# matter-labs/era-zkevm_test_harness

Hardware: AMD Instinct MI355X
Metric: base-layer circuits/sec (2^20 rows); full-block synth wall-time 1/8 GPU (higher is better)
Workload: dtype u64 (Goldilocks, p = 2^64 - 2^32 + 1)

## Files before the change

era_zkevm_test_harness_amd/csrc/ram_circuit_kernels.cuh:

```cuda
#pragma once
#include "../../include/zkw_ram_circuit_spec.h"
#include "../../include/zkw_decommit_sorter_circuit_spec.h"
#include "../../include/zkw_events_sorter_circuit_spec.h"
#include "ram_kernels.cuh"
#include "public_input_kernels.cuh"
#include "closed_form_kernels.cuh"

namespace zkw {

struct SynthJob {
    const zkw_ram_instance* inst;
    const zkw_mem_query* sorted_q;
    const zkw_mem_query* unsorted_q;
    const u64* unsorted_caps;
    const u64* sorted_caps;
    const u64* u_mark;
    const u64* s_mark;
    const u64* challenges;
    const u64* lhs_z;
    const u64* rhs_z;
    u64 n_block;
    u64* trace;
    u32* hist;
    u32* nd_tiles;
    const u64* public_input;
    const zkw_ram_instance* first_inst;
    u32 tail_clean;
};

constexpr int ROW_SLOTS[RC_NUM_ROW_TYPES] = RC_ROW_NUM_SLOTS_INIT;
constexpr int ROW_LOOKUPS[RC_NUM_ROW_TYPES] = RC_ROW_NUM_LOOKUPS_INIT;
static_assert(ROW_SLOTS[RC_ROW_PU] == 133 && ROW_SLOTS[RC_ROW_PS] == 130, "Poseidon2 rows: 130 gate variables (+3 spare in PU)");
static_assert(ROW_LOOKUPS[RC_ROW_PU] == 12 && ROW_LOOKUPS[RC_ROW_PS] == 12 && ROW_LOOKUPS[RC_ROW_A] == 12 &&
              ROW_LOOKUPS[RC_ROW_B] == 12 && ROW_LOOKUPS[RC_ROW_C] == 8 && ROW_LOOKUPS[RC_ROW_D] == 0,
              "lookup cells per cycle (56) are hard-wired in the fill kernels");
constexpr int LOOKUPS_PER_CYCLE = 56;

__device__ __forceinline__ u64 inv_or_zero(u64 x) { return gl::canon(x) ? gl::inv(x) : 0; }

struct RegsIn {
    const u64* uh;
    const u64* sh;
    u32 len;
};
// ... 79 lines not shown
    memset(&c.q, 0, sizeof c.q);
    memset(&c.pq, 0, sizeof c.pq);
#pragma unroll
    for (int k = 0; k < 8; k++) c.es[k] = 0;
    if (c.can_pop) {
        load_query(job.sorted_q + first + i, c.q);
        encode_mem_query(c.q, c.es);
    }
    if (i == 0) {
        const zkw_ram_fsm& f = in->hidden_fsm_input;
        c.pq.timestamp = f.previous_sorting_key[0]; c.pq.index = f.previous_sorting_key[1]; c.pq.page = f.previous_sorting_key[2];
        for (int k = 0; k < 8; k++) c.pq.value[k] = f.previous_value[k];
        c.pq.value_is_pointer = f.previous_is_ptr ? 1 : 0;
    } else if (i - 1 < m) {
        load_query(job.sorted_q + first + i - 1, c.pq);
    }
    u64 pe[8];
    encode_mem_query(c.pq, pe);
#pragma unroll
    for (int k = 0; k < 5; k++) c.p_val[k] = pe[3 + k];
    c.p_ptr = c.pq.value_is_pointer ? 1 : 0;
}

__device__ __forceinline__ u64 acc_before(const u64* z, size_t first, size_t m, u32 i, u64 fsm_in) {
    return i == 0 ? fsm_in : z[first + (i - 1 < m ? i - 1 : m - 1)];
}

__device__ __forceinline__ void fill_row_A(const SynthJob& job, u32 i, u32 capacity, size_t n_rows, const zkw_mem_query& q,
                                           const u64 eu[8], const u64 es[8], u32* sh_hist) {
    u64* trace = job.trace;
    const size_t row = (size_t)RC_ROW_A * RC_REGION_STRIDE(capacity) + i;
    if (i < capacity) {
        const zkw_ram_instance* in = job.inst;
        const size_t first = in->first_item, m = in->num_items, n_total = job.n_block;
        const bool can_pop = i < m;
        const u64 rw = q.rw_flag ? 1 : 0, ptr = q.value_is_pointer ? 1 : 0;
#pragma unroll
        for (int k = 0; k < 8; k++) { TR(RC_A_eu0 + k, row) = eu[k]; TR(RC_A_ts + k, row) = es[k]; }
        for (int r = 0; r < 2; r++) {
            const u64* ch = job.challenges + 9 * r;
            u64 lc = ch[8], rc = ch[8];
#pragma unroll
            for (int k = 0; k < 8; k++) {
                lc = gl::add(lc, gl::mul(eu[k], ch[k]));
                rc = gl::add(rc, gl::mul(es[k], ch[k]));
                __builtin_amdgcn_sched_barrier(0);
            }
            const u64 pl = acc_before(job.lhs_z + (size_t)r * n_total, first, m, i, in->hidden_fsm_input.lhs_accumulator[r]);
            const u64 pr = acc_before(job.rhs_z + (size_t)r * n_total, first, m, i, in->hidden_fsm_input.rhs_accumulator[r]);
            const u64 nl = gl::canon(gl::mul(pl, lc)), nr = gl::canon(gl::mul(pr, rc));
            const int o = r * (RC_A_lc1 - RC_A_lc0);
#pragma unroll
            for (int k = 1; k < 9; k++) TR(RC_A_G_c0_1 + (k - 1) + r * (RC_A_G_c1_1 - RC_A_G_c0_1), row) = ch[k];
            __builtin_amdgcn_sched_barrier(0);
            TR(RC_A_lc0 + o, row) = gl::canon(lc); TR(RC_A_P_lhs0 + o, row) = pl; TR(RC_A_nl0 + o, row) = nl;
            TR(RC_A_lhs0 + o, row) = can_pop ? nl : pl;
            TR(RC_A_rc0 + o, row) = gl::canon(rc); TR(RC_A_P_rhs0 + o, row) = pr; TR(RC_A_nr0 + o, row) = nr;
            TR(RC_A_rhs0 + o, row) = can_pop ? nr : pr;
            __builtin_amdgcn_sched_barrier(0);
        }
        TR(RC_A_rw, row) = rw; TR(RC_A_ptr, row) = ptr; TR(RC_A_idx, row) = q.index;
        TR(RC_A_v2, row) = q.value[2]; TR(RC_A_v3, row) = q.value[3]; TR(RC_A_v0, row) = q.value[0];
        TR(RC_A_v5_b3c, row) = q.value[5] >> 24; TR(RC_A_can_pop, row) = can_pop ? 1 : 0;
        put_bytes(trace, n_rows, row, RC_A_v2_b0, q.value[2]);
        put_bytes(trace, n_rows, row, RC_A_v3_b0, q.value[3]);
        put_bytes(trace, n_rows, row, RC_A_v5_b0, q.value[5]);
        hist_bytes(sh_hist, q.value[2]); hist_bytes(sh_hist, q.value[3]); hist_bytes(sh_hist, q.value[5]);
        constexpr int NA = ROW_SLOTS[RC_ROW_A];
        if (!job.tail_clean) {
            for (int col = NA; col < RC_G; col++) TR(col, row) = 0;
            for (int col = RC_G + 12; col < RC_G + RC_L; col++) TR(col, row) = 0;
        }
    } else if (i < RC_REGION_STRIDE(capacity)) {
        if (!job.tail_clean) zero_gap_row(trace, n_rows, row);
    }
}

__device__ __forceinline__ void fill_row_B(const SynthJob& job, u32 i, u32 capacity, size_t n_rows, const zkw_mem_query& q,
                                           const u64 es[8], u32* sh_hist) {
    u64* trace = job.trace;
    const size_t row = (size_t)RC_ROW_B * RC_REGION_STRIDE(capacity) + i;
    if (i < capacity) {
        const zkw_ram_instance* in = job.inst;
// ... 286 lines not shown
        const size_t per = (n_pairs + TAIL_CHUNKS - 1) / TAIL_CHUNKS, lo = ch * per, hi = lo + per < n_pairs ? lo + per : n_pairs;
        ulonglong2* c2 = reinterpret_cast<ulonglong2*>(trace + (size_t)col * n_rows + bnd);
        const ulonglong2 z = make_ulonglong2(0, 0);
        for (size_t k = lo + threadIdx.x; k < hi; k += 256) c2[k] = z;
        return;
    }
    u64* m = trace + (size_t)RC_MULT_COL * n_rows;
    const size_t per = (n_rows + TAIL_CHUNKS - 1) / TAIL_CHUNKS, lo = ch * per, hi = lo + per < n_rows ? lo + per : n_rows;
    for (size_t r = lo + threadIdx.x; r < (job.tail_clean && hi > 256 ? (lo < 256 ? 256 : lo) : hi); r += 256) {
        u64 v = 0;
        if (r < 256) {
            v = job.hist[r];
            if (r == 0) v += (u64)RC_L * n_rows - (u64)LOOKUPS_PER_CYCLE * capacity - RC_CF_LOOKUP_CELLS;
        }
        m[r] = v;
    }
}

static __constant__ rc_link c_links[RC_NUM_LINKS] = RC_LINKS_INIT;
static __constant__ uint8_t c_is_poseidon[RC_NUM_ROW_TYPES] = RC_ROW_IS_POSEIDON_INIT;
ZKW_CF_TABLES(RC, rc)

__device__ __forceinline__ void ram_fill_register_rows(const SynthJob& job, u32 capacity, size_t n_rows) {
    const u64* lhs_z_all = job.lhs_z;
    const u64* rhs_z_all = job.rhs_z;
    const size_t n_total = job.n_block;
    u64* trace = job.trace;
    const zkw_ram_instance* in = job.inst;
    const zkw_ram_fsm& fi = in->hidden_fsm_input;
    const size_t first = in->first_item, m = in->num_items;
    const size_t bin = (size_t)RC_BOUNDARY_ROW(capacity) + RC_ROWOFF_BND_IN, bout = bin - RC_ROWOFF_BND_IN + RC_ROWOFF_BND_OUT;
    const RegsIn ri = regs_in(in);
    for (int k = 0; k < 12; k++) { TR(RC_BND_IN_uh0 + k, bin) = ri.uh[k]; TR(RC_BND_IN_sh0 + k, bin) = ri.sh[k]; }
    TR(RC_BND_IN_len_u, bin) = ri.len; TR(RC_BND_IN_len_s, bin) = ri.len;
    for (int r = 0; r < 2; r++) { TR(RC_BND_IN_lhs0 + r, bin) = fi.lhs_accumulator[r]; TR(RC_BND_IN_rhs0 + r, bin) = fi.rhs_accumulator[r]; }
    zkw_mem_query pq;
    memset(&pq, 0, sizeof pq);
    for (int k = 0; k < 8; k++) pq.value[k] = fi.previous_value[k];
    u64 pe[8];
    encode_mem_query(pq, pe);
    TR(RC_BND_IN_ts, bin) = fi.previous_sorting_key[0]; TR(RC_BND_IN_idx, bin) = fi.previous_sorting_key[1];
    TR(RC_BND_IN_page, bin) = fi.previous_sorting_key[2];
    TR(RC_BND_IN_es3, bin) = pe[3]; TR(RC_BND_IN_es4, bin) = pe[4]; TR(RC_BND_IN_es5, bin) = pe[5];
    TR(RC_BND_IN_es6, bin) = pe[6]; TR(RC_BND_IN_v4, bin) = pe[7];
    TR(RC_BND_IN_ptr, bin) = fi.previous_is_ptr ? 1 : 0; TR(RC_BND_IN_cnt, bin) = fi.num_nondeterministic_writes;
    for (int r = 0; r < 2; r++)
        for (int k = 1; k < 9; k++) TR(RC_BND_IN_G_c0_1 + 8 * r + (k - 1), bin) = job.challenges[9 * r + k];
    const size_t last = first + m - 1;
    const bool padded = m < capacity;
    const u64 len_out = (u64)ri.len - m;
    for (int k = 0; k < 12; k++) {
        TR(RC_BND_OUT_uh0 + k, bout) = job.u_mark[k];
        TR(RC_BND_OUT_sh0 + k, bout) = job.s_mark[k];
        TR(RC_BND_OUT_tail_u0 + k, bout) = in->unsorted_queue_initial_state.tail[k];
        TR(RC_BND_OUT_tail_s0 + k, bout) = in->sorted_queue_initial_state.tail[k];
    }
    TR(RC_BND_OUT_len_u, bout) = len_out; TR(RC_BND_OUT_len_s, bout) = len_out;
    for (int r = 0; r < 2; r++) {
        TR(RC_BND_OUT_lhs0 + r, bout) = lhs_z_all[(size_t)r * n_total + last];
        TR(RC_BND_OUT_rhs0 + r, bout) = rhs_z_all[(size_t)r * n_total + last];
    }
    zkw_mem_query lq;
    memset(&lq, 0, sizeof lq);
    if (!padded) lq = job.sorted_q[last];
    u64 le[8];
    encode_mem_query(lq, le);
    TR(RC_BND_OUT_ts, bout) = lq.timestamp; TR(RC_BND_OUT_idx, bout) = lq.index; TR(RC_BND_OUT_page, bout) = lq.page;
    TR(RC_BND_OUT_es3, bout) = le[3]; TR(RC_BND_OUT_es4, bout) = le[4]; TR(RC_BND_OUT_es5, bout) = le[5];
    TR(RC_BND_OUT_es6, bout) = le[6]; TR(RC_BND_OUT_v4, bout) = le[7];
    TR(RC_BND_OUT_ptr, bout) = lq.value_is_pointer ? 1 : 0;
    TR(RC_BND_OUT_cnt, bout) = TR(RC_C_cnt, (size_t)RC_ROW_C * RC_REGION_STRIDE(capacity) + capacity - 1);
    TR(RC_BND_OUT_completion, bout) = in->completion_flag ? 1 : 0;
    TR(RC_BND_OUT_w_end, bout) = inv_or_zero(len_out); TR(RC_BND_OUT_z_end, bout) = len_out == 0;
}

__device__ __forceinline__ void ram_value_row(u64* trace, size_t n_rows, size_t row, int v0, int b0, int e3) {
    zkw_mem_query q;
    memset(&q, 0, sizeof q);
    for (int k = 0; k < 8; k++) q.value[k] = (u32)TR(v0 + k, row);
    for (int l = 5; l < 8; l++)
        for (int k = 0; k < 4; k++) {
            const u64 b = (q.value[l] >> (8 * k)) & 0xFF;
            TR(b0 + 4 * (l - 5) + k, row) = b;
// ... 225 lines not shown
```

era_zkevm_test_harness_amd/csrc/ram_kernels.cuh:

```cuda
#pragma once
#include "../../include/zkw_types.h"
#include "poseidon2.cuh"

namespace zkw {
using gl::u32;
using gl::u64;

__device__ __forceinline__ void encode_mem_query(const zkw_mem_query& q, u64 out[8]) {
    const u32* v = q.value;
    out[0] = q.timestamp;
    out[1] = q.page;
    out[2] = (u64)q.index | ((u64)(q.rw_flag ? 1 : 0) << 32) | ((u64)(q.value_is_pointer ? 1 : 0) << 33);
    u64 b5 = v[5], b6 = v[6], b7 = v[7];
    out[3] = (u64)v[0] | ((b5 & 0xFFFFFF) << 32);
    out[4] = (u64)v[1] | ((b5 >> 24) << 32) | ((b6 & 0xFFFF) << 40);
    out[5] = (u64)v[2] | ((b6 >> 16) << 32) | ((b7 & 0xFF) << 48);
    out[6] = (u64)v[3] | ((b7 >> 8) << 32);
    out[7] = v[4];
}

static __device__ __forceinline__ void k_encode_mem(const VB& vb, const zkw_mem_query* __restrict__ q, size_t n,
                                                    u64* __restrict__ enc) {
    size_t i = (size_t)vb.x * blockDim.x + threadIdx.x;
    size_t stride = (size_t)vb.nx * blockDim.x;
// ... 415 lines not shown
    uint4 w0 = src[0], w1 = src[1], w2 = src[2];
    uint4* dq = reinterpret_cast<uint4*>(sorted_q + i);
    dq[0] = w0; dq[1] = w1; dq[2] = w2;
    zkw_mem_query m;
    uint4* dm = reinterpret_cast<uint4*>(&m);
    dm[0] = w0; dm[1] = w1; dm[2] = w2;
    if (!sorted_enc) return;
    u64 e[8];
    encode_mem_query(m, e);
    ulonglong2* o = reinterpret_cast<ulonglong2*>(sorted_enc + 8 * i);
    o[0] = make_ulonglong2(e[0], e[1]); o[1] = make_ulonglong2(e[2], e[3]);
    o[2] = make_ulonglong2(e[4], e[5]); o[3] = make_ulonglong2(e[6], e[7]);
}

struct RamBlock {
    const zkw_mem_query* sorted_q;
    const u32* sorted_perm;
    const u64* u_marks;
    const u64* s_marks;
    const u64* lhs_z;
    const u64* rhs_z;
    zkw_ram_instance* instances;
    u32* nondet_prefix;
    u64 n;
    u32 capacity;
    u32 num_nondet_heap_queries;
};

__device__ __forceinline__ void copy12(u64* dst, const u64* src) {
    for (int k = 0; k < 12; k++) dst[k] = src[k];
}

static __device__ __forceinline__ void k_ram_count_nondet(const VB& vb, const RamBlock* __restrict__ blocks) {
    const RamBlock b = blocks[vb.y];
    const u64 n_inst = (b.n + b.capacity - 1) / b.capacity;
    __shared__ u32 sh[4];
    for (u64 inst = vb.x; inst < n_inst; inst += vb.nx) {
        const u64 lo = inst * b.capacity, hi = lo + b.capacity < b.n ? lo + b.capacity : b.n;
        u32 cnt = 0;
        for (u64 i = lo + threadIdx.x; i < hi; i += blockDim.x) {
            const zkw_mem_query* q = b.sorted_q + b.sorted_perm[i];
            cnt += (q->rw_flag && q->timestamp == 0 && q->page == ZKW_BOOTLOADER_HEAP_PAGE) ? 1u : 0u;
        }
        for (int d = 32; d > 0; d >>= 1) cnt += __shfl_down(cnt, d, 64);
        if ((threadIdx.x & 63) == 0) sh[threadIdx.x >> 6] = cnt;
        __syncthreads();
// ... 36 lines not shown
        f.current_sorted_queue_state.length = (u32)(n - end);
        const zkw_mem_query* q = b.sorted_q + b.sorted_perm[l];
        f.previous_sorting_key[0] = q->timestamp; f.previous_sorting_key[1] = q->index; f.previous_sorting_key[2] = q->page;
        f.previous_full_key[0] = q->index; f.previous_full_key[1] = q->page;
        for (int k = 0; k < 8; k++) f.previous_value[k] = q->value[k];
        f.previous_is_ptr = q->value_is_pointer ? 1 : 0;
        f.num_nondeterministic_writes = nondet;
    };
    if (idx == 0) {
        for (int r = 0; r < 2; r++) { w.hidden_fsm_input.lhs_accumulator[r] = 1; w.hidden_fsm_input.rhs_accumulator[r] = 1; }
    } else {
        fill(w.hidden_fsm_input, lo, nondet_before);
    }
    fill(w.hidden_fsm_output, hi, nondet_before + b.nondet_prefix[idx]);
    if ((hi - lo) % b.capacity != 0) {
        zkw_ram_fsm& f = w.hidden_fsm_output;
        for (int k = 0; k < 3; k++) f.previous_sorting_key[k] = 0;
        for (int k = 0; k < 2; k++) f.previous_full_key[k] = 0;
        for (int k = 0; k < 8; k++) f.previous_value[k] = 0;
        f.previous_is_ptr = 0;
    }
}


static __device__ __forceinline__ void k_tails_expand(const VB& vb, const u64* __restrict__ enc, const u64* __restrict__ caps,
                                                     const u64* __restrict__ offsets, int n_queues, size_t n,
                                                     u64* __restrict__ tails) {
    const size_t i = (size_t)vb.x * blockDim.x + threadIdx.x;
    if (i >= n) return;
    int lo = 0, hi = n_queues;
    while (hi - lo > 1) {
        const int mid = (lo + hi) >> 1;
        if (offsets[mid] <= i) lo = mid; else hi = mid;
    }
    u64 s[12];
#pragma unroll
    for (int k = 0; k < 8; k++) s[k] = enc[8 * i + k];
    const bool first = offsets[lo] == i;
#pragma unroll
    for (int k = 0; k < 4; k++) s[8 + k] = first ? 0 : caps[4 * (i - 1) + k];
    p2::permute(s);
#pragma unroll
    for (int k = 0; k < 12; k++) tails[12 * i + k] = gl::canon(s[k]);
}

}
// ... 1 lines not shown
```

era_zkevm_test_harness_amd/csrc/zkw_api.hip:

```cpp
#include "zkw_ctx.h"
#include "circuit_check_host.h"
#include "closed_forms_host.h"
#include "callstack_kernels.cuh"
#include "vm_kernels.cuh"
#include "radix_sort.cuh"

static thread_local std::string g_last_error;

#undef fail
int zkw_fail(int code, const char* fmt, ...) {
    char buf[512];
    va_list ap;
    va_start(ap, fmt);
    vsnprintf(buf, sizeof buf, fmt, ap);
    va_end(ap);
    g_last_error = buf;
    return code;
}

#define fail zkw_fail

struct AllocCache {
    static constexpr size_t SMALL_MAX = size_t(256) << 20;
    static constexpr int MAX_DEV = 16;
// ... 912 lines not shown
    uint64_t offsets[2] = {0, n};
    return zkw_queue_push_chain_log_batch(ctx, enc, offsets, 1, tail_in, old_tails, new_tails);
}

struct zkw_ram_witness {
    zkw_ctx* ctx = nullptr;
    std::vector<uint64_t> offsets;
    std::vector<uint64_t> inst_offsets;
    uint32_t capacity = 0;
    size_t total = 0, n_instances = 0;
    zkw_mem_query* sorted_q = nullptr;
    bool sorted_valid = false;
    u32* perm = nullptr;
    const zkw_mem_query* unsorted_q = nullptr;
    zkw_mem_query* owned_q = nullptr;
    u64 *unsorted_enc = nullptr, *sorted_enc = nullptr;
    bool enc_valid = false;
    u64 *unsorted_caps = nullptr, *sorted_caps = nullptr, *unsorted_marks = nullptr, *sorted_marks = nullptr;
    u64 *unsorted_tails = nullptr, *sorted_tails = nullptr;
    bool tails_valid = false;
    u64 *challenges = nullptr, *lhs_z = nullptr, *rhs_z = nullptr;
    bool z_valid = false;
    u64 *zbuf_l = nullptr, *zbuf_r = nullptr;
    zkw_mem_query* sq_win = nullptr;
    size_t zcap = 0, sqcap = 0;
    zkw_ram_instance* instances = nullptr;
    u32* nondet_counts = nullptr;
    u64 *compact_forms = nullptr, *public_inputs = nullptr;

    void release() {
        void* ptrs[] = {sorted_q, perm, owned_q, unsorted_enc, sorted_enc, unsorted_caps, sorted_caps, unsorted_marks, sorted_marks,
                        unsorted_tails, sorted_tails, challenges,
                        lhs_z,    rhs_z,        instances,  nondet_counts, compact_forms, public_inputs, zbuf_l, zbuf_r, sq_win};
        for (void* p : ptrs)
            if (p) dev_free(p);
        sorted_q = nullptr;
        sorted_valid = false;
        perm = nullptr;
        owned_q = nullptr;
        unsorted_q = nullptr;
        enc_valid = false;
        unsorted_enc = sorted_enc = unsorted_tails = sorted_tails = challenges = lhs_z = rhs_z = nullptr;
        unsorted_caps = sorted_caps = unsorted_marks = sorted_marks = nullptr;
        tails_valid = false;
        z_valid = false;
        zbuf_l = zbuf_r = nullptr;
        sq_win = nullptr;
        zcap = sqcap = 0;
        instances = nullptr;
        nondet_counts = nullptr;
        compact_forms = public_inputs = nullptr;
    }
};

extern "C" void zkw_ram_witness_free(zkw_ram_witness* w);
static int ram_alloc(zkw_ram_witness* w, size_t n_blocks) {
    const size_t t = w->total, ni = w->n_instances;
    HIP_TRY(dev_malloc((void**)&w->perm, (t + 1) * sizeof(u32)));
    HIP_TRY(dev_malloc((void**)&w->unsorted_caps, (t + 1) * 4 * sizeof(u64)));
    HIP_TRY(dev_malloc((void**)&w->sorted_caps, (t + 1) * 4 * sizeof(u64)));
    HIP_TRY(dev_malloc((void**)&w->unsorted_marks, (ni + 1) * 12 * sizeof(u64)));
    HIP_TRY(dev_malloc((void**)&w->sorted_marks, (ni + 1) * 12 * sizeof(u64)));
    HIP_TRY(dev_malloc((void**)&w->challenges, (n_blocks + 1) * 18 * sizeof(u64)));
    {
        size_t max_block = 0;
        for (size_t b = 0; b + 1 < w->offsets.size(); b++) max_block = std::max(max_block, (size_t)(w->offsets[b + 1] - w->offsets[b]));
        size_t window = (size_t)1 << 26, sq_window = (size_t)1 << 22;
        if (const char* e = getenv("ZKW_Z_WINDOW_ITEMS")) window = sq_window = (size_t)strtoull(e, nullptr, 10);
        w->zcap = std::max(max_block, std::min(t, window));
        w->sqcap = std::max(max_block, std::min(t, sq_window));
        HIP_TRY(dev_malloc((void**)&w->zbuf_l, (w->zcap + 1) * 2 * sizeof(u64)));
        HIP_TRY(dev_malloc((void**)&w->zbuf_r, (w->zcap + 1) * 2 * sizeof(u64)));
        HIP_TRY(dev_malloc((void**)&w->sq_win, (w->sqcap + 1) * sizeof(zkw_mem_query)));
    }
    HIP_TRY(dev_malloc((void**)&w->instances, (ni + 1) * sizeof(zkw_ram_instance)));
    HIP_TRY(dev_malloc((void**)&w->nondet_counts, (ni + 1) * sizeof(u32)));
    HIP_TRY(dev_malloc((void**)&w->compact_forms, (ni + 1) * COMPACT_FORM_LEN * sizeof(u64)));
    HIP_TRY(dev_malloc((void**)&w->public_inputs, (ni + 1) * 4 * sizeof(u64)));
    return ZKW_OK;
}

__device__ __forceinline__ u32 block_of_position(const u64* __restrict__ offsets, int n_blocks, size_t i) {
    int lo = 0, hi = n_blocks;
    while (hi - lo > 1) {
        int mid = (lo + hi) >> 1;
        if (offsets[mid] <= i) lo = mid; else hi = mid;
    }
    return (u32)lo;
}

static __device__ __forceinline__ void k_ram_key_ranges(const VB& vb, const zkw_mem_query* __restrict__ q, size_t n, u32* __restrict__ maxima) {
    u32 t = 0, p = 0, x = 0;
    for (size_t i = (size_t)vb.x * blockDim.x + threadIdx.x; i < n; i += (size_t)vb.nx * blockDim.x) {
        t = max(t, q[i].timestamp);
        p = max(p, q[i].page);
        x = max(x, q[i].index);
    }
// ... 151 lines not shown
                      w->challenges + 18 * b};
    }
    ZKW_TRY(dev_fs(ctx, fs, 12, 9));
    w->z_valid = false;
    for (size_t b0 = 0; b0 < n_blocks;) {
        size_t b1 = b0 + 1;
        while (b1 < n_blocks && w->offsets[b1 + 1] - w->offsets[b0] <= w->zcap) b1++;
        ZKW_TRY(ram_gp_blocks(ctx, w, b0, b1, w->zbuf_l, w->zbuf_r));
        const size_t base = w->offsets[b0];
        std::vector<RamBlock> blocks(b1 - b0);
        size_t max_inst = 0;
        for (size_t b = b0; b < b1; b++) {
            const size_t lo = w->offsets[b], n = w->offsets[b + 1] - lo;
            const size_t n_inst = w->inst_offsets[b + 1] - w->inst_offsets[b];
            if (n_inst > max_inst) max_inst = n_inst;
            blocks[b - b0] = RamBlock{w->unsorted_q,
                                      w->perm + lo,
                                      w->unsorted_marks + 12 * w->inst_offsets[b],
                                      w->sorted_marks + 12 * w->inst_offsets[b],
                                      w->zbuf_l + 2 * (lo - base),
                                      w->zbuf_r + 2 * (lo - base),
                                      w->instances + w->inst_offsets[b],
                                      w->nondet_counts + w->inst_offsets[b],
                                      n,
                                      w->capacity,
                                      n_nondet ? n_nondet[b] : 0u};
        }
        RamBlock* d_blocks = nullptr;
        ZKW_TRY(ctx->upload("ram_blocks", blocks, &d_blocks));
        const unsigned gx = (unsigned)(max_inst < 64 ? max_inst : 64), gy = (unsigned)(b1 - b0);
        { Prof _p(ctx, "k_ram_count_nondet"); ZKW_LAUNCH_2D(ctx, k_ram_count_nondet, gx, gy, 256, d_blocks); }
        ZKW_TRY(launch_check("k_ram_count_nondet"));
        { Prof _p(ctx, "k_ram_instances"); ZKW_LAUNCH_2D(ctx, k_ram_instances, blocks_for(max_inst, 64), gy, 64, d_blocks); }
        ZKW_TRY(launch_check("k_ram_instances"));
        b0 = b1;
    }
    const size_t ni = w->n_instances;
    { Prof _p(ctx, "k_ram_commitments"); ZKW_LAUNCH(ctx, k_ram_commitments, blocks_for(4 * ni, 64), 64, w->instances, ni, w->compact_forms); }
    ZKW_TRY(launch_check("k_ram_commitments"));
    { Prof _p(ctx, "k_commit_encodings"); ZKW_LAUNCH(ctx, k_commit_encodings, blocks_for(ni, 64), 64, w->compact_forms, ni, (u32)COMPACT_FORM_LEN, w->public_inputs); }
    return launch_check("k_commit_encodings");
}

extern "C" int zkw_ram_build_instances_batch(zkw_ctx* ctx, const zkw_mem_query* q, const uint64_t* block_offsets,
                                             size_t n_blocks, uint32_t capacity, const uint32_t* n_nondet,
                                             zkw_ram_witness** out) {
    if (!ctx || !q || !block_offsets || !out || n_blocks == 0 || capacity == 0)
        return fail(ZKW_ERR_INVALID, "zkw_ram_build_instances_batch: bad argument");
    HIP_TRY(hipSetDevice(ctx->device));
    const uint64_t base = block_offsets[0];
    std::vector<uint64_t> offs(n_blocks + 1), ioffs(n_blocks + 1, 0);
    for (size_t b = 0; b <= n_blocks; b++) offs[b] = block_offsets[b] - base;
    for (size_t b = 0; b < n_blocks; b++) {
        if (block_offsets[b + 1] <= block_offsets[b])
            return fail(ZKW_ERR_INVALID, "block %zu is empty: the VM must have made memory requests "
                                         "(W/ram_permutation.rs:43-46)", b);
        ioffs[b + 1] = ioffs[b] + (offs[b + 1] - offs[b] + capacity - 1) / capacity;
// ... 111 lines not shown
    { Prof _p(ctx, "k_tails_expand"); ZKW_LAUNCH(ctx, k_tails_expand, blocks_for(t, 64), 64, w->sorted_enc, w->sorted_caps, d_off, nq, t, w->sorted_tails); }
    ZKW_TRY(launch_check("k_tails_expand"));
    w->tails_valid = true;
    return ZKW_OK;
}

static const void* ram_array(const zkw_ram_witness* w, int what, size_t* bytes, bool materialize = true, int* rc = nullptr) {
    const size_t t = w->total, nb = w->offsets.size() - 1;
    int st = ZKW_OK;
    const void* p = nullptr;
#define RAM_LAZY(fn, field) do { if (materialize) { st = fn(w); if (st == ZKW_OK) p = w->field; } } while (0)
    switch (what) {
        case ZKW_RAM_SORTED_QUERIES: *bytes = t * sizeof(zkw_mem_query); RAM_LAZY(ram_sorted_queries, sorted_q); break;
        case ZKW_RAM_UNSORTED_ENC: *bytes = t * 64; RAM_LAZY(ram_encodings, unsorted_enc); break;
        case ZKW_RAM_SORTED_ENC: *bytes = t * 64; RAM_LAZY(ram_encodings, sorted_enc); break;
        case ZKW_RAM_UNSORTED_TAILS: *bytes = t * 96; RAM_LAZY(ram_full_tails, unsorted_tails); break;
        case ZKW_RAM_SORTED_TAILS: *bytes = t * 96; RAM_LAZY(ram_full_tails, sorted_tails); break;
        case ZKW_RAM_CHALLENGES: *bytes = nb * 18 * 8; p = w->challenges; break;
        case ZKW_RAM_LHS_Z: *bytes = t * 16; RAM_LAZY(ram_full_chains, lhs_z); break;
        case ZKW_RAM_RHS_Z: *bytes = t * 16; RAM_LAZY(ram_full_chains, rhs_z); break;
        case ZKW_RAM_INSTANCES: *bytes = w->n_instances * sizeof(zkw_ram_instance); p = w->instances; break;
        case ZKW_RAM_COMPACT_FORMS: *bytes = w->n_instances * COMPACT_FORM_LEN * 8; p = w->compact_forms; break;
        case ZKW_RAM_PUBLIC_INPUTS: *bytes = w->n_instances * 32; p = w->public_inputs; break;
        default: *bytes = 0; st = ZKW_ERR_INVALID; break;
    }
#undef RAM_LAZY
    if (rc) *rc = st;
    return p;
}

extern "C" size_t zkw_ram_witness_bytes(const zkw_ram_witness* w, int what) {
    size_t b = 0;
    if (w) (void)ram_array(w, what, &b, false);
    return b;
}

extern "C" const void* zkw_ram_witness_device_ptr(const zkw_ram_witness* w, int what) {
    size_t b = 0;
    return w ? ram_array(w, what, &b) : nullptr;
}

extern "C" int zkw_ram_witness_get(const zkw_ram_witness* w, int what, void* dst, size_t dst_bytes) {
    if (!w || !dst) return fail(ZKW_ERR_INVALID, "zkw_ram_witness_get: null argument");
    size_t bytes = 0;
    int st = ZKW_OK;
    const void* src = ram_array(w, what, &bytes, true, &st);
// ... 69 lines not shown
    const u64* src = t->data + slot * t->slot_elems() + (size_t)first_col * t->n_rows;
    HIP_TRY(ctx->copy_async(dst, src, (size_t)n_cols * t->n_rows * sizeof(u64), ctx->ptr_mode == ZKW_PTR_DEVICE ? hipMemcpyDeviceToDevice : hipMemcpyDeviceToHost));
    return ctx->sync_if_host();
}

extern "C" int zkw_ram_synthesize(zkw_ctx* ctx, const zkw_ram_witness* w, size_t first_instance, size_t n_instances,
                                  zkw_trace* t, size_t first_slot) {
    if (!ctx || !w || !t || w->ctx != ctx || t->ctx->device != ctx->device) return fail(ZKW_ERR_INVALID, "zkw_ram_synthesize: bad argument");
    if (first_instance + n_instances > w->n_instances) return fail(ZKW_ERR_INVALID, "instance range out of bounds");
    if (n_instances > t->n_slots) return fail(ZKW_ERR_INVALID, "more instances (%zu) than trace slots (%zu)", n_instances, t->n_slots);
    const u32 capacity = w->capacity;
    const size_t n_rows = t->n_rows;
    if (RC_MIN_ROWS(capacity) > n_rows)
        return fail(ZKW_ERR_INVALID, "capacity %u needs %llu rows, trace has %zu", capacity,
                    (unsigned long long)RC_MIN_ROWS(capacity), n_rows);
    if (n_rows & 1) return fail(ZKW_ERR_INVALID, "trace length must be even (it is a power of two in every circuit)");
    if (n_instances == 0) return ZKW_OK;
    HIP_TRY(hipSetDevice(ctx->device));
    const size_t n_blocks = w->offsets.size() - 1;
    size_t b_first = 0;
    while (b_first + 1 < n_blocks && w->inst_offsets[b_first + 1] <= first_instance) b_first++;
    size_t b_end = b_first + 1;
    while (b_end < n_blocks && w->inst_offsets[b_end] < first_instance + n_instances) b_end++;
    const size_t win = std::min(w->zcap, w->sqcap);
    if (w->offsets[b_end] - w->offsets[b_first] > win) {
        size_t b_mid = b_first + 1;
        while (b_mid + 1 < b_end && w->offsets[b_mid + 1] - w->offsets[b_first] <= win) b_mid++;
        const size_t n_head = w->inst_offsets[b_mid] - first_instance;
        ZKW_TRY(zkw_ram_synthesize(ctx, w, first_instance, n_head, t, first_slot));
        return zkw_ram_synthesize(ctx, w, first_instance + n_head, n_instances - n_head, t, first_slot + n_head);
    }
    ZKW_TRY(ram_gp_blocks(ctx, w, b_first, b_end, w->zbuf_l, w->zbuf_r));
    const size_t z_base = w->offsets[b_first];
    {
        const size_t cnt = w->offsets[b_end] - z_base;
        Prof _p(ctx, "k_gather_encode");
        ZKW_LAUNCH(ctx, k_gather_encode, blocks_for(cnt, 256), 256, w->unsorted_q, w->perm + z_base, cnt, w->sq_win, (u64*)nullptr);
    }
    ZKW_TRY(launch_check("k_gather_encode"));
    const u32 rstride = (u32)RC_REGION_STRIDE(capacity);
    const u32 n_tiles = (rstride + 255) / 256;
    u32 *d_hist = nullptr, *d_nd = nullptr;
    ZKW_TRY(ctx->scratch_t<u32>("synth_hist", n_instances * 256, &d_hist));
    ZKW_TRY(ctx->scratch_t<u32>("synth_nd", n_instances * n_tiles, &d_nd));
    HIP_TRY(ctx->memset_async(d_hist, 0, n_instances * 256 * sizeof(u32)));
    SlotClaims claims(t);
    std::vector<SynthJob> jobs(n_instances);
    size_t b = b_first;
    for (size_t k = 0; k < n_instances; k++) {
        const size_t idx = first_instance + k;
        while (b + 1 < n_blocks && w->inst_offsets[b + 1] <= idx) b++;
        const size_t lo = w->offsets[b], nb = w->offsets[b + 1] - lo;
        SynthJob& j = jobs[k];
        j.inst = w->instances + idx;
        j.sorted_q = w->sq_win + (lo - z_base);
        j.unsorted_q = w->unsorted_q + lo;
        j.unsorted_caps = w->unsorted_caps + 4 * lo;
        j.sorted_caps = w->sorted_caps + 4 * lo;
        j.u_mark = w->unsorted_marks + 12 * idx;
        j.s_mark = w->sorted_marks + 12 * idx;
        j.challenges = w->challenges + 18 * b;
        j.lhs_z = w->zbuf_l + 2 * (lo - z_base);
        j.rhs_z = w->zbuf_r + 2 * (lo - z_base);
        j.n_block = nb;
        {
            const uint64_t tag = ((uint64_t)ZKW_CIRCUIT_RAM_PERMUTATION << 56) ^ ((uint64_t)capacity << 24) ^ (uint64_t)n_rows ^ 0x5A00000000000000ull;
            const size_t slot = (first_slot + k) % t->n_slots;
            bool clean = false;
            j.trace = claims.claim(slot, tag, &clean);
            j.tail_clean = clean;
        }
        j.hist = d_hist + 256 * k;
        j.nd_tiles = d_nd + (size_t)n_tiles * k;
        j.public_input = w->public_inputs + 4 * idx;
        j.first_inst = w->instances + w->inst_offsets[b];
    }
    SynthJob* d_jobs = nullptr;
    ZKW_TRY(ctx->upload("synth_jobs", jobs, &d_jobs));
    const unsigned nj = (unsigned)n_instances;
    const dim3 g64((rstride + 63) / 64, nj), g256(n_tiles, nj);
    { Prof _p(ctx, "k_ram_nd_tiles"); ZKW_LAUNCH_D(ctx, (k_ram_nd_tiles), "k_ram_nd_tiles", g256, 256, 0, d_jobs, capacity); }
    ZKW_TRY(launch_check("k_ram_nd_tiles"));
    { Prof _p(ctx, "k_ram_nd_scan"); ZKW_LAUNCH(ctx, k_ram_nd_scan, nj, 64, d_jobs, (int)nj, n_tiles); }
    ZKW_TRY(launch_check("k_ram_nd_scan"));
    { Prof _p(ctx, "k_ram_fill_poseidon"); ZKW_LAUNCH_D(ctx, (k_ram_fill_poseidon<0>), "k_ram_fill_poseidon", g64, 64, 0, d_jobs, capacity, n_rows); }
    ZKW_TRY(launch_check("k_ram_fill_poseidon<0>"));
    { Prof _p(ctx, "k_ram_fill_poseidon"); ZKW_LAUNCH_D(ctx, (k_ram_fill_poseidon<1>), "k_ram_fill_poseidon", g64, 64, 0, d_jobs, capacity, n_rows); }
// ... 224 lines not shown
```

era_zkevm_test_harness_amd/native.py:

```python
import ctypes as C
import os

os.environ.setdefault("GPU_MAX_HW_QUEUES", "8")

import numpy as np

_HERE = os.path.dirname(os.path.abspath(__file__))
LIB_PATH = os.environ.get("ZKW_LIB", os.path.join(_HERE, "libzkw.so"))

OK, ERR_INVALID, ERR_NO_DEVICE, ERR_HIP, ERR_OOM, ERR_CHECK_FAILED = 0, -1, -2, -3, -4, -5
PTR_HOST, PTR_DEVICE = 0, 1
(RAM_SORTED_QUERIES, RAM_UNSORTED_ENC, RAM_SORTED_ENC, RAM_UNSORTED_TAILS, RAM_SORTED_TAILS, RAM_CHALLENGES,
 RAM_LHS_Z, RAM_RHS_Z, RAM_INSTANCES, RAM_COMPACT_FORMS, RAM_PUBLIC_INPUTS) = range(11)

_vp, _sz, _u32, _u64p, _int = C.c_void_p, C.c_size_t, C.c_uint32, C.c_void_p, C.c_int
SYMBOLS = [
    ("zkw_process_init", _int, []),
    ("zkw_create", _vp, [_int]),
    ("zkw_destroy", None, [_vp]),
    ("zkw_last_error", C.c_char_p, []),
    ("zkw_set_stream", _int, [_vp, _vp]),
    ("zkw_set_chain_stream", _int, [_vp, _vp]),
    ("zkw_set_pointer_mode", _int, [_vp, _int]),
    ("zkw_synchronize", _int, [_vp]),
    ("zkw_set_chain_form", _int, [_vp, _int]),
    ("zkw_set_netlist_fill_form", _int, [_vp, _int]),
    ("zkw_set_chain_service", _int, [_vp, _int]),
    ("zkw_set_chain_tag", _int, [_vp, _int]),
    ("zkw_chain_service_expect", _int, [_int, _int]),
    ("zkw_buffer_alloc", _int, [_vp, _int, C.c_size_t, C.POINTER(C.c_void_p)]),
    ("zkw_buffer_free", None, [_int, _vp]),
    ("zkw_stream_acquire", _int, [_vp, C.POINTER(C.c_void_p)]),
    ("zkw_stream_release", None, [_vp, _vp]),
    ("zkw_trim_caches", None, []),
    ("zkw_block_linear_hasher_instance", _int, [_vp, _vp]),
    ("zkw_setup_copy_permutation", _int, [C.c_uint8, C.c_uint32, _sz, _vp, _vp]),
# ... 937 lines not shown
    def num_items(self):
        return load().zkw_ram_witness_num_items(self.handle)

    def device_ptr(self, what):
        return load().zkw_ram_witness_device_ptr(self.handle, what)

    def nbytes(self, what):
        return load().zkw_ram_witness_bytes(self.handle, what)

    def get(self, what):
        lib = load()
        nbytes = lib.zkw_ram_witness_bytes(self.handle, what)
        dt = self._DTYPES.get(what, np.dtype("<u8"))
        out = np.zeros(nbytes // dt.itemsize, dt)
        mode = self.ctx.pointer_mode
        self.ctx.set_pointer_mode(PTR_HOST)
        try:
            _check(lib.zkw_ram_witness_get(self.handle, what, _np_ptr(out), nbytes))
        finally:
            self.ctx.set_pointer_mode(mode)
        t = self.num_items
        shape = {RAM_UNSORTED_ENC: (t, 8), RAM_SORTED_ENC: (t, 8), RAM_UNSORTED_TAILS: (t, 12),
                 RAM_SORTED_TAILS: (t, 12), RAM_CHALLENGES: (-1, 2, 9), RAM_COMPACT_FORMS: (-1, 18),
                 RAM_PUBLIC_INPUTS: (-1, 4)}.get(what)
        return out.reshape(shape) if shape else out

    def free(self):
        if self.handle:
            load().zkw_ram_witness_free(self.handle)
            self.handle = C.c_void_p(None)

    def __del__(self):
        try:
            self.free()
        except Exception:
            pass


class Trace:

    def __init__(self, ctx, n_rows, n_slots=1, n_cols=None):
        self.ctx = ctx
        self.handle = C.c_void_p(None)
        if n_cols is None:
            _check(load().zkw_trace_create(ctx.handle, n_rows, n_slots, C.byref(self.handle)))
        else:
            _check(load().zkw_trace_create_with_columns(ctx.handle, n_rows, n_cols, n_slots, C.byref(self.handle)))
# ... 1264 lines not shown
```

include/zkw.h:

```cpp
#ifndef ZKW_H
#define ZKW_H
#include "zkw_types.h"

#ifdef __cplusplus
extern "C" {
#endif

typedef struct zkw_ctx zkw_ctx;
typedef struct zkw_ram_witness zkw_ram_witness;
typedef struct zkw_trace zkw_trace;

enum {
    ZKW_OK = 0,
    ZKW_ERR_INVALID = -1,
    ZKW_ERR_NO_DEVICE = -2,
    ZKW_ERR_HIP = -3,
    ZKW_ERR_OOM = -4,
    ZKW_ERR_CHECK_FAILED = -5
};

enum { ZKW_PTR_HOST = 0, ZKW_PTR_DEVICE = 1 };

int zkw_process_init(void);
zkw_ctx *zkw_create(int device_id);
// ... 104 lines not shown
int zkw_fs_challenges(zkw_ctx *ctx, const uint64_t *tail_u, uint32_t len_u, const uint64_t *tail_s,
                      uint32_t len_s, int state_w, int n_chal, uint64_t *out);

int zkw_grand_product_chains(zkw_ctx *ctx, const uint64_t *lhs, const uint64_t *rhs, size_t n, int width,
                             const uint64_t *challenges, int n_reps, uint64_t *lhs_z, uint64_t *rhs_z);

int zkw_ram_build_instances(zkw_ctx *ctx, const zkw_mem_query *q, size_t n, uint32_t capacity,
                            uint32_t num_non_deterministic_heap_queries, zkw_ram_witness **out);
int zkw_ram_build_instances_batch(zkw_ctx *ctx, const zkw_mem_query *q, const uint64_t *block_offsets,
                                  size_t n_blocks, uint32_t capacity, const uint32_t *n_nondet,
                                  zkw_ram_witness **out);

enum {
    ZKW_RAM_SORTED_QUERIES = 0,
    ZKW_RAM_UNSORTED_ENC = 1,
    ZKW_RAM_SORTED_ENC = 2,
    ZKW_RAM_UNSORTED_TAILS = 3,
    ZKW_RAM_SORTED_TAILS = 4,
    ZKW_RAM_CHALLENGES = 5,
    ZKW_RAM_LHS_Z = 6,
    ZKW_RAM_RHS_Z = 7,
    ZKW_RAM_INSTANCES = 8,
    ZKW_RAM_COMPACT_FORMS = 9,
    ZKW_RAM_PUBLIC_INPUTS = 10
};
size_t zkw_ram_witness_num_instances(const zkw_ram_witness *w);
size_t zkw_ram_witness_num_items(const zkw_ram_witness *w);
size_t zkw_ram_witness_bytes(const zkw_ram_witness *w, int what);
const void *zkw_ram_witness_device_ptr(const zkw_ram_witness *w, int what);
int zkw_ram_witness_get(const zkw_ram_witness *w, int what, void *dst, size_t dst_bytes);
void zkw_ram_witness_free(zkw_ram_witness *w);

typedef struct zkw_decommit_witness zkw_decommit_witness;
int zkw_decommit_sorter_build(zkw_ctx *ctx, const zkw_decommit_query *q, size_t n, uint32_t capacity,
                              const zkw_queue_state12 *dedup_in, zkw_decommit_witness **out);
int zkw_decommit_sorter_prepare(zkw_ctx *ctx, const zkw_decommit_query *q, size_t n, uint32_t capacity,
                                const zkw_queue_state12 *dedup_in, zkw_decommit_witness **out);
int zkw_decommit_sorter_finish(zkw_ctx *ctx, zkw_decommit_witness *w);
enum {
    ZKW_DEC_SORTED_QUERIES = 0,
    ZKW_DEC_UNSORTED_ENC = 1,
    ZKW_DEC_SORTED_ENC = 2,
    ZKW_DEC_UNSORTED_TAILS = 3,
    ZKW_DEC_SORTED_TAILS = 4,
    ZKW_DEC_DEDUP_QUERIES = 5,
    ZKW_DEC_DEDUP_TAILS = 6,
    ZKW_DEC_CHALLENGES = 7,
// ... 458 lines not shown
```

Baseline: 3263.

## Recompute grand-product accumulators in-wavefront from per-64-row checkpoints instead of reading z arrays

Instead of materialising the full lhs/rhs grand-product z arrays per synthesis window and reading one value per row, the witness build now stores a checkpoint accumulator every 64 rows per instance. Row-A fill rebuilds each row's prior accumulator with a wavefront-wide multiplicative prefix scan using shuffles, seeded from the checkpoint. The boundary output row now reads the instance's hidden FSM output. This drops the per-window ram_gp_blocks pass and its z-buffer traffic, and the window is no longer limited by the z buffer. In exchange, row-A threads do about 12 extra field multiplies and shuffles, every lane including dead ones now takes part in the scan, and one small checkpoint kernel is added.

```diff
diff --git a/era_zkevm_test_harness_amd/csrc/ram_circuit_kernels.cuh b/era_zkevm_test_harness_amd/csrc/ram_circuit_kernels.cuh
--- a/era_zkevm_test_harness_amd/csrc/ram_circuit_kernels.cuh
+++ b/era_zkevm_test_harness_amd/csrc/ram_circuit_kernels.cuh
@@ -17,9 +17,7 @@
     const u64* u_mark;
     const u64* s_mark;
     const u64* challenges;
-    const u64* lhs_z;
-    const u64* rhs_z;
-    u64 n_block;
+    const u64* gp_ckpt;
     u64* trace;
     u32* hist;
     u32* nd_tiles;
@@ -145,32 +143,43 @@
     c.p_ptr = c.pq.value_is_pointer ? 1 : 0;
 }
 
-__device__ __forceinline__ u64 acc_before(const u64* z, size_t first, size_t m, u32 i, u64 fsm_in) {
-    return i == 0 ? fsm_in : z[first + (i - 1 < m ? i - 1 : m - 1)];
+__device__ __forceinline__ void acc_before_pair(u64 fl, u64 fr, u64 ckpt_l, u64 ckpt_r, int lane, u64& pl, u64& pr) {
+#pragma unroll
+    for (int d = 1; d < 64; d <<= 1) {
+        const u64 ol = __shfl_up(fl, d, 64), orr = __shfl_up(fr, d, 64);
+        if (lane >= d) { fl = gl::mul(fl, ol); fr = gl::mul(fr, orr); }
+        __builtin_amdgcn_sched_barrier(0);
+    }
+    const u64 el = __shfl_up(fl, 1, 64), er = __shfl_up(fr, 1, 64);
+    pl = lane == 0 ? ckpt_l : gl::canon(gl::mul(ckpt_l, el));
+    pr = lane == 0 ? ckpt_r : gl::canon(gl::mul(ckpt_r, er));
+    __builtin_amdgcn_sched_barrier(0);
 }
 
 __device__ __forceinline__ void fill_row_A(const SynthJob& job, u32 i, u32 capacity, size_t n_rows, const zkw_mem_query& q,
                                            const u64 eu[8], const u64 es[8], u32* sh_hist) {
     u64* trace = job.trace;
     const size_t row = (size_t)RC_ROW_A * RC_REGION_STRIDE(capacity) + i;
-    if (i < capacity) {
-        const zkw_ram_instance* in = job.inst;
-        const size_t first = in->first_item, m = in->num_items, n_total = job.n_block;
-        const bool can_pop = i < m;
-        const u64 rw = q.rw_flag ? 1 : 0, ptr = q.value_is_pointer ? 1 : 0;
+    const bool live = i < capacity;
+    const bool can_pop = live && i < job.inst->num_items;
+    const int lane = threadIdx.x & 63;
+    const u64* ckpt = job.gp_ckpt + 4 * (size_t)((u32)__builtin_amdgcn_readfirstlane((int)i) >> 6);
+    if (live) {
 #pragma unroll
         for (int k = 0; k < 8; k++) { TR(RC_A_eu0 + k, row) = eu[k]; TR(RC_A_ts + k, row) = es[k]; }
-        for (int r = 0; r < 2; r++) {
-            const u64* ch = job.challenges + 9 * r;
-            u64 lc = ch[8], rc = ch[8];
-#pragma unroll
-            for (int k = 0; k < 8; k++) {
-                lc = gl::add(lc, gl::mul(eu[k], ch[k]));
-                rc = gl::add(rc, gl::mul(es[k], ch[k]));
-                __builtin_amdgcn_sched_barrier(0);
-            }
-            const u64 pl = acc_before(job.lhs_z + (size_t)r * n_total, first, m, i, in->hidden_fsm_input.lhs_accumulator[r]);
-            const u64 pr = acc_before(job.rhs_z + (size_t)r * n_total, first, m, i, in->hidden_fsm_input.rhs_accumulator[r]);
+    }
+    for (int r = 0; r < 2; r++) {
+        const u64* ch = job.challenges + 9 * r;
+        u64 lc = ch[8], rc = ch[8];
+#pragma unroll
+        for (int k = 0; k < 8; k++) {
+            lc = gl::add(lc, gl::mul(eu[k], ch[k]));
+            rc = gl::add(rc, gl::mul(es[k], ch[k]));
+            __builtin_amdgcn_sched_barrier(0);
+        }
+        u64 pl, pr;
+        acc_before_pair(can_pop ? lc : 1, can_pop ? rc : 1, ckpt[r], ckpt[2 + r], lane, pl, pr);
+        if (live) {
             const u64 nl = gl::canon(gl::mul(pl, lc)), nr = gl::canon(gl::mul(pr, rc));
             const int o = r * (RC_A_lc1 - RC_A_lc0);
 #pragma unroll
@@ -180,8 +189,11 @@
             TR(RC_A_lhs0 + o, row) = can_pop ? nl : pl;
             TR(RC_A_rc0 + o, row) = gl::canon(rc); TR(RC_A_P_rhs0 + o, row) = pr; TR(RC_A_nr0 + o, row) = nr;
             TR(RC_A_rhs0 + o, row) = can_pop ? nr : pr;
-            __builtin_amdgcn_sched_barrier(0);
-        }
+        }
+        __builtin_amdgcn_sched_barrier(0);
+    }
+    if (live) {
+        const u64 rw = q.rw_flag ? 1 : 0, ptr = q.value_is_pointer ? 1 : 0;
         TR(RC_A_rw, row) = rw; TR(RC_A_ptr, row) = ptr; TR(RC_A_idx, row) = q.index;
         TR(RC_A_v2, row) = q.value[2]; TR(RC_A_v3, row) = q.value[3]; TR(RC_A_v0, row) = q.value[0];
         TR(RC_A_v5_b3c, row) = q.value[5] >> 24; TR(RC_A_can_pop, row) = can_pop ? 1 : 0;
@@ -514,9 +526,6 @@
 ZKW_CF_TABLES(RC, rc)
 
 __device__ __forceinline__ void ram_fill_register_rows(const SynthJob& job, u32 capacity, size_t n_rows) {
-    const u64* lhs_z_all = job.lhs_z;
-    const u64* rhs_z_all = job.rhs_z;
-    const size_t n_total = job.n_block;
     u64* trace = job.trace;
     const zkw_ram_instance* in = job.inst;
     const zkw_ram_fsm& fi = in->hidden_fsm_input;
@@ -549,8 +558,8 @@
     }
     TR(RC_BND_OUT_len_u, bout) = len_out; TR(RC_BND_OUT_len_s, bout) = len_out;
     for (int r = 0; r < 2; r++) {
-        TR(RC_BND_OUT_lhs0 + r, bout) = lhs_z_all[(size_t)r * n_total + last];
-        TR(RC_BND_OUT_rhs0 + r, bout) = rhs_z_all[(size_t)r * n_total + last];
+        TR(RC_BND_OUT_lhs0 + r, bout) = in->hidden_fsm_output.lhs_accumulator[r];
+        TR(RC_BND_OUT_rhs0 + r, bout) = in->hidden_fsm_output.rhs_accumulator[r];
     }
     zkw_mem_query lq;
     memset(&lq, 0, sizeof lq);
diff --git a/era_zkevm_test_harness_amd/csrc/ram_kernels.cuh b/era_zkevm_test_harness_amd/csrc/ram_kernels.cuh
--- a/era_zkevm_test_harness_amd/csrc/ram_kernels.cuh
+++ b/era_zkevm_test_harness_amd/csrc/ram_kernels.cuh
@@ -461,6 +461,7 @@
     const u64* rhs_z;
     zkw_ram_instance* instances;
     u32* nondet_prefix;
+    u64* gp_ckpt;
     u64 n;
     u32 capacity;
     u32 num_nondet_heap_queries;
@@ -543,6 +544,21 @@
     }
 }
 
+static __device__ __forceinline__ void k_ram_gp_ckpt(const VB& vb, const RamBlock* __restrict__ blocks) {
+    const RamBlock b = blocks[vb.y];
+    const u64 n_inst = (b.n + b.capacity - 1) / b.capacity, groups = (b.capacity + 63) / 64;
+    const u64 j = (u64)vb.x * blockDim.x + threadIdx.x;
+    if (j >= n_inst * groups) return;
+    const u64 idx = j / groups, g = j % groups;
+    const zkw_ram_instance& in = b.instances[idx];
+    const u64 first = in.first_item, m = in.num_items;
+    u64* out = b.gp_ckpt + 4 * j;
+    for (int r = 0; r < 2; r++) {
+        const u64 at = (u64)r * b.n + first + (64 * g - 1 < m ? 64 * g - 1 : m - 1);
+        out[r] = g == 0 ? in.hidden_fsm_input.lhs_accumulator[r] : b.lhs_z[at];
+        out[2 + r] = g == 0 ? in.hidden_fsm_input.rhs_accumulator[r] : b.rhs_z[at];
+    }
+}
 
 static __device__ __forceinline__ void k_tails_expand(const VB& vb, const u64* __restrict__ enc, const u64* __restrict__ caps,
                                                      const u64* __restrict__ offsets, int n_queues, size_t n,
diff --git a/era_zkevm_test_harness_amd/csrc/zkw_api.hip b/era_zkevm_test_harness_amd/csrc/zkw_api.hip
--- a/era_zkevm_test_harness_amd/csrc/zkw_api.hip
+++ b/era_zkevm_test_harness_amd/csrc/zkw_api.hip
@@ -958,6 +958,7 @@
     u64 *challenges = nullptr, *lhs_z = nullptr, *rhs_z = nullptr;
     bool z_valid = false;
     u64 *zbuf_l = nullptr, *zbuf_r = nullptr;
+    u64* gp_ckpt = nullptr;
     zkw_mem_query* sq_win = nullptr;
     size_t zcap = 0, sqcap = 0;
     zkw_ram_instance* instances = nullptr;
@@ -967,7 +968,7 @@
     void release() {
         void* ptrs[] = {sorted_q, perm, owned_q, unsorted_enc, sorted_enc, unsorted_caps, sorted_caps, unsorted_marks, sorted_marks,
                         unsorted_tails, sorted_tails, challenges,
-                        lhs_z,    rhs_z,        instances,  nondet_counts, compact_forms, public_inputs, zbuf_l, zbuf_r, sq_win};
+                        lhs_z,    rhs_z,        instances,  nondet_counts, compact_forms, public_inputs, zbuf_l, zbuf_r, sq_win, gp_ckpt};
         for (void* p : ptrs)
             if (p) dev_free(p);
         sorted_q = nullptr;
@@ -981,6 +982,7 @@
         tails_valid = false;
         z_valid = false;
         zbuf_l = zbuf_r = nullptr;
+        gp_ckpt = nullptr;
         sq_win = nullptr;
         zcap = sqcap = 0;
         instances = nullptr;
@@ -990,6 +992,7 @@
 };
 
 extern "C" void zkw_ram_witness_free(zkw_ram_witness* w);
+static inline size_t ram_gp_groups(uint32_t capacity) { return ((size_t)capacity + 63) / 64; }
 static int ram_alloc(zkw_ram_witness* w, size_t n_blocks) {
     const size_t t = w->total, ni = w->n_instances;
     HIP_TRY(dev_malloc((void**)&w->perm, (t + 1) * sizeof(u32)));
@@ -1009,6 +1012,7 @@
         HIP_TRY(dev_malloc((void**)&w->zbuf_r, (w->zcap + 1) * 2 * sizeof(u64)));
         HIP_TRY(dev_malloc((void**)&w->sq_win, (w->sqcap + 1) * sizeof(zkw_mem_query)));
     }
+    HIP_TRY(dev_malloc((void**)&w->gp_ckpt, (ni * ram_gp_groups(w->capacity) + 1) * 4 * sizeof(u64)));
     HIP_TRY(dev_malloc((void**)&w->instances, (ni + 1) * sizeof(zkw_ram_instance)));
     HIP_TRY(dev_malloc((void**)&w->nondet_counts, (ni + 1) * sizeof(u32)));
     HIP_TRY(dev_malloc((void**)&w->compact_forms, (ni + 1) * COMPACT_FORM_LEN * sizeof(u64)));
@@ -1206,6 +1210,7 @@
                                       w->zbuf_r + 2 * (lo - base),
                                       w->instances + w->inst_offsets[b],
                                       w->nondet_counts + w->inst_offsets[b],
+                                      w->gp_ckpt + 4 * ram_gp_groups(w->capacity) * w->inst_offsets[b],
                                       n,
                                       w->capacity,
                                       n_nondet ? n_nondet[b] : 0u};
@@ -1217,6 +1222,8 @@
         ZKW_TRY(launch_check("k_ram_count_nondet"));
         { Prof _p(ctx, "k_ram_instances"); ZKW_LAUNCH_2D(ctx, k_ram_instances, blocks_for(max_inst, 64), gy, 64, d_blocks); }
         ZKW_TRY(launch_check("k_ram_instances"));
+        { Prof _p(ctx, "k_ram_gp_ckpt"); ZKW_LAUNCH_2D(ctx, k_ram_gp_ckpt, blocks_for(max_inst * ram_gp_groups(w->capacity), 256), gy, 256, d_blocks); }
+        ZKW_TRY(launch_check("k_ram_gp_ckpt"));
         b0 = b1;
     }
     const size_t ni = w->n_instances;
@@ -1374,6 +1381,7 @@
         case ZKW_RAM_INSTANCES: *bytes = w->n_instances * sizeof(zkw_ram_instance); p = w->instances; break;
         case ZKW_RAM_COMPACT_FORMS: *bytes = w->n_instances * COMPACT_FORM_LEN * 8; p = w->compact_forms; break;
         case ZKW_RAM_PUBLIC_INPUTS: *bytes = w->n_instances * 32; p = w->public_inputs; break;
+        case ZKW_RAM_GP_CKPT: *bytes = w->n_instances * ram_gp_groups(w->capacity) * 32; p = w->gp_ckpt; break;
         default: *bytes = 0; st = ZKW_ERR_INVALID; break;
     }
 #undef RAM_LAZY
@@ -1489,7 +1497,7 @@
     while (b_first + 1 < n_blocks && w->inst_offsets[b_first + 1] <= first_instance) b_first++;
     size_t b_end = b_first + 1;
     while (b_end < n_blocks && w->inst_offsets[b_end] < first_instance + n_instances) b_end++;
-    const size_t win = std::min(w->zcap, w->sqcap);
+    const size_t win = w->sqcap;
     if (w->offsets[b_end] - w->offsets[b_first] > win) {
         size_t b_mid = b_first + 1;
         while (b_mid + 1 < b_end && w->offsets[b_mid + 1] - w->offsets[b_first] <= win) b_mid++;
@@ -1497,7 +1505,6 @@
         ZKW_TRY(zkw_ram_synthesize(ctx, w, first_instance, n_head, t, first_slot));
         return zkw_ram_synthesize(ctx, w, first_instance + n_head, n_instances - n_head, t, first_slot + n_head);
     }
-    ZKW_TRY(ram_gp_blocks(ctx, w, b_first, b_end, w->zbuf_l, w->zbuf_r));
     const size_t z_base = w->offsets[b_first];
     {
         const size_t cnt = w->offsets[b_end] - z_base;
@@ -1517,7 +1524,7 @@
     for (size_t k = 0; k < n_instances; k++) {
         const size_t idx = first_instance + k;
         while (b + 1 < n_blocks && w->inst_offsets[b + 1] <= idx) b++;
-        const size_t lo = w->offsets[b], nb = w->offsets[b + 1] - lo;
+        const size_t lo = w->offsets[b];
         SynthJob& j = jobs[k];
         j.inst = w->instances + idx;
         j.sorted_q = w->sq_win + (lo - z_base);
@@ -1527,9 +1534,7 @@
         j.u_mark = w->unsorted_marks + 12 * idx;
         j.s_mark = w->sorted_marks + 12 * idx;
         j.challenges = w->challenges + 18 * b;
-        j.lhs_z = w->zbuf_l + 2 * (lo - z_base);
-        j.rhs_z = w->zbuf_r + 2 * (lo - z_base);
-        j.n_block = nb;
+        j.gp_ckpt = w->gp_ckpt + 4 * ram_gp_groups(capacity) * idx;
         {
             const uint64_t tag = ((uint64_t)ZKW_CIRCUIT_RAM_PERMUTATION << 56) ^ ((uint64_t)capacity << 24) ^ (uint64_t)n_rows ^ 0x5A00000000000000ull;
             const size_t slot = (first_slot + k) % t->n_slots;
diff --git a/era_zkevm_test_harness_amd/native.py b/era_zkevm_test_harness_amd/native.py
--- a/era_zkevm_test_harness_amd/native.py
+++ b/era_zkevm_test_harness_amd/native.py
@@ -11,7 +11,7 @@
 OK, ERR_INVALID, ERR_NO_DEVICE, ERR_HIP, ERR_OOM, ERR_CHECK_FAILED = 0, -1, -2, -3, -4, -5
 PTR_HOST, PTR_DEVICE = 0, 1
 (RAM_SORTED_QUERIES, RAM_UNSORTED_ENC, RAM_SORTED_ENC, RAM_UNSORTED_TAILS, RAM_SORTED_TAILS, RAM_CHALLENGES,
- RAM_LHS_Z, RAM_RHS_Z, RAM_INSTANCES, RAM_COMPACT_FORMS, RAM_PUBLIC_INPUTS) = range(11)
+ RAM_LHS_Z, RAM_RHS_Z, RAM_INSTANCES, RAM_COMPACT_FORMS, RAM_PUBLIC_INPUTS, RAM_GP_CKPT) = range(12)
 
 _vp, _sz, _u32, _u64p, _int = C.c_void_p, C.c_size_t, C.c_uint32, C.c_void_p, C.c_int
 SYMBOLS = [
@@ -995,7 +995,7 @@
         t = self.num_items
         shape = {RAM_UNSORTED_ENC: (t, 8), RAM_SORTED_ENC: (t, 8), RAM_UNSORTED_TAILS: (t, 12),
                  RAM_SORTED_TAILS: (t, 12), RAM_CHALLENGES: (-1, 2, 9), RAM_COMPACT_FORMS: (-1, 18),
-                 RAM_PUBLIC_INPUTS: (-1, 4)}.get(what)
+                 RAM_PUBLIC_INPUTS: (-1, 4), RAM_GP_CKPT: (self.num_instances, -1, 4)}.get(what)
         return out.reshape(shape) if shape else out
 
     def free(self):
diff --git a/include/zkw.h b/include/zkw.h
--- a/include/zkw.h
+++ b/include/zkw.h
@@ -150,7 +150,8 @@
     ZKW_RAM_RHS_Z = 7,
     ZKW_RAM_INSTANCES = 8,
     ZKW_RAM_COMPACT_FORMS = 9,
-    ZKW_RAM_PUBLIC_INPUTS = 10
+    ZKW_RAM_PUBLIC_INPUTS = 10,
+    ZKW_RAM_GP_CKPT = 11
 };
 size_t zkw_ram_witness_num_instances(const zkw_ram_witness *w);
 size_t zkw_ram_witness_num_items(const zkw_ram_witness *w);
```

Result: faster. 3447 (median of 6 runs) (+5.6%).
